# xiexh20/VisTracker

Measured on AMD Instinct MI355X. Metric: frames/sec joint SMPL+object fit, higher is better.
Workload: dtype f32 (decoder GEMMs: 22-bit split-f16 operands x3 MFMA, fp32 accumulate)

## Files before the change

include/vistracker.h:

```cpp
#ifndef VISTRACKER_H
#define VISTRACKER_H

#ifdef __cplusplus
extern "C" {
#endif

#define VT_OK 0
#define VT_ERR_ARG -1
#define VT_ERR_HIP -2
#define VT_ERR_BUSY -3

#define VT_SMPL_V 6890
#define VT_SMPL_J 52
#define VT_SMPL_NB 10
#define VT_SMPL_NP 459
#define VT_FEAT 611
#define VT_HID 128

const char *vt_last_error(void);
int vt_version(void);

typedef struct vt_smplh vt_smplh;

int vt_smplh_create(vt_smplh **out, const float *v_template, const float *shapedirs, const float *posedirs,
                    const float *J_regressor, const float *weights, const int *parents, void *stream);
void vt_smplh_destroy(vt_smplh *h);

long vt_smplh_workspace_floats(int B);

int vt_smplh_forward(const vt_smplh *h, const float *pose, const float *betas, const float *trans, int B,
                     float *verts, float *jtr, float *v_posed, float *ws, void *stream);

long vt_smplh_bwd_scratch_floats(int B);
int vt_smplh_backward(const vt_smplh *h, const float *pose, const float *betas, int B, const float *dverts,
                      const float *djtr, const float *v_posed, const float *ws, float *scratch,
                      float *dpose, float *dbetas, float *dtrans, void *stream);

long vt_smplh_prefix_floats(int B);
int vt_smplh_prefix(const vt_smplh *h, const float *pose, int B, float *ws, float *prefix, void *stream);
int vt_smplh_forward_prefixed(const vt_smplh *h, const float *pose, const float *betas, const float *trans, int B, const float *prefix,
                              float *verts, float *jtr, float *v_posed, float *ws, void *stream);
int vt_smplh_backward_free(const vt_smplh *h, const float *pose, int B, const float *dverts, const float *djtr, const float *v_posed,
                           const float *ws, float *scratch, int n_free_pose_cols, float *dpose, float *dbetas, float *dtrans, void *stream);

int vt_rodrigues_forward(const float *aa, int n, float *R, void *stream);
int vt_rodrigues_backward(const float *aa, int n, const float *dR, float *daa, void *stream);

typedef struct vt_landmarks vt_landmarks;
int vt_landmarks_create(vt_landmarks **out, const int *indptr, const int *indices, const float *data, int K, int V,
                        void *stream);
void vt_landmarks_destroy(vt_landmarks *h);
int vt_landmarks_forward(const vt_landmarks *h, const float *verts, int B, float *out, void *stream);
int vt_landmarks_backward(const vt_landmarks *h, const float *dout, int B, float *dverts, int accumulate, void *stream);

int vt_mahalanobis(const float *x, int B, int stride, int off, int n, const float *mean, const float *prec,
                   float *value, float *dx, float gscale, void *stream);

int vt_fill_f64(double *p, long n, double value, void *stream);
int vt_sum_to_term(const float *value, int n, float scale, double *term, void *stream);

typedef struct vt_sifnet vt_sifnet;
int vt_sifnet_create(vt_sifnet **out, const float *const *w, const float *const *b, const float *cam, void *stream);
void vt_sifnet_destroy(vt_sifnet *h);

int vt_nchw_to_nhwc(const float *src, int B, int C, int H, int W, float *dst, void *stream);

typedef struct {
    const float *maps[8];
    int res[8];
    const float *proj;
    int proj_cols;
    int act_level;
    int proj_level;
    int force_fp32;
} vt_maps;

int vt_query_forward(const vt_sifnet *h, const vt_maps *maps, const float *pts, const float *crop_center,
                     const float *body_center, int B, int N,
                     float *df, float *pca, float *parts, float *centers, float *vis, void *stream);
int vt_query_backward(const vt_sifnet *h, const vt_maps *maps, const float *pts, const float *crop_center,
                      const float *body_center, int B, int N,
                      const float *d_df, const float *d_pca, const float *d_parts, const float *d_centers,
                      const float *d_vis, float *dpts, void *stream);

long vt_query_projection_floats(const vt_maps *maps, int B);
int vt_query_build_projection(const vt_sifnet *h, const vt_maps *maps, int B, float *proj, void *stream);

int vt_query_human_loss(const vt_sifnet *h, const vt_maps *maps, const float *pts, const float *crop_center,
                        const float *body_center, int B, int N, const int *labels, const int *order, float w_dfh, float w_part,
                        float *dpts, double *terms, void *stream);
int vt_query_object_loss(const vt_sifnet *h, const vt_maps *maps, const float *pts, const float *crop_center,
                         const float *body_center, int B, int N, const float *occ, float w_obj,
                         float *dpts, double *terms, void *stream);

typedef struct vt_conv3x3 vt_conv3x3;
int vt_conv3x3_create(vt_conv3x3 **out, const float *weight, int cout, int cin, void *stream);
// ... 263 lines not shown
```

vistracker_amd/_lib.py:

```python
from __future__ import annotations

import ctypes as C
import os

_HERE = os.path.dirname(os.path.abspath(__file__))
LIB_PATH = os.environ.get("VT_LIB_PATH", os.path.join(_HERE, "libvistracker_hip.so"))

vp = C.c_void_p
fp = C.c_void_p
ci = C.c_int
cl = C.c_long
cf = C.c_float
cd = C.c_double


class VtMaps(C.Structure):
    _fields_ = [("maps", C.c_void_p * 8), ("res", C.c_int * 8), ("proj", C.c_void_p), ("proj_cols", C.c_int),
                ("act_level", C.c_int), ("proj_level", C.c_int), ("force_fp32", C.c_int)]


SIGNATURES = {
    "vt_last_error": (C.c_char_p, []),
    "vt_version": (ci, []),
    "vt_smplh_create": (ci, [C.POINTER(vp), vp, vp, vp, vp, vp, vp, vp]),
    "vt_smplh_destroy": (None, [vp]),
    "vt_smplh_workspace_floats": (cl, [ci]),
    "vt_smplh_bwd_scratch_floats": (cl, [ci]),
    "vt_smplh_forward": (ci, [vp, fp, fp, fp, ci, fp, fp, fp, fp, vp]),
    "vt_smplh_backward": (ci, [vp, fp, fp, ci, fp, fp, fp, fp, fp, fp, fp, fp, vp]),
    "vt_smplh_prefix_floats": (cl, [ci]),
    "vt_smplh_prefix": (ci, [vp, fp, ci, fp, fp, vp]),
    "vt_smplh_forward_prefixed": (ci, [vp, fp, fp, fp, ci, fp, fp, fp, fp, fp, vp]),
    "vt_smplh_backward_free": (ci, [vp, fp, ci, fp, fp, fp, fp, fp, ci, fp, fp, fp, vp]),
    "vt_rodrigues_forward": (ci, [fp, ci, fp, vp]),
    "vt_rodrigues_backward": (ci, [fp, ci, fp, fp, vp]),
    "vt_landmarks_create": (ci, [C.POINTER(vp), vp, vp, vp, ci, ci, vp]),
    "vt_landmarks_destroy": (None, [vp]),
    "vt_landmarks_forward": (ci, [vp, fp, ci, fp, vp]),
    "vt_landmarks_backward": (ci, [vp, fp, ci, fp, ci, vp]),
    "vt_mahalanobis": (ci, [fp, ci, ci, ci, ci, fp, fp, fp, fp, cf, vp]),
    "vt_fill_f64": (ci, [fp, cl, cd, vp]),
    "vt_sum_to_term": (ci, [fp, ci, cf, fp, vp]),
    "vt_sifnet_create": (ci, [C.POINTER(vp), C.POINTER(vp), C.POINTER(vp), vp, vp]),
    "vt_sifnet_destroy": (None, [vp]),
    "vt_nchw_to_nhwc": (ci, [fp, ci, ci, ci, ci, fp, vp]),
    "vt_query_forward": (ci, [vp, C.POINTER(VtMaps), fp, fp, fp, ci, ci, fp, fp, fp, fp, fp, vp]),
    "vt_query_backward": (ci, [vp, C.POINTER(VtMaps), fp, fp, fp, ci, ci, fp, fp, fp, fp, fp, fp, vp]),
    "vt_query_human_loss": (ci, [vp, C.POINTER(VtMaps), fp, fp, fp, ci, ci, fp, fp, cf, cf, fp, fp, vp]),
    "vt_query_object_loss": (ci, [vp, C.POINTER(VtMaps), fp, fp, fp, ci, ci, fp, cf, fp, fp, vp]),
    "vt_query_set_human_kernel": (ci, [ci]),
    "vt_sifnet_set_precision": (ci, [vp, ci]),
    "vt_sifnet_get_precision": (ci, [vp]),
    "vt_groupnorm_nhwc": (ci, [fp, fp, fp, ci, ci, ci, ci, cf, ci, fp, fp, vp]),
    "vt_upsample2x_bicubic_add": (ci, [fp, fp, ci, ci, ci, ci, fp, vp]),
    "vt_conv3x3_create": (ci, [C.POINTER(vp), vp, ci, ci, vp]),
    "vt_conv3x3_destroy": (None, [vp]),
    "vt_conv3x3_forward": (ci, [vp, fp, ci, ci, ci, fp, ci, ci, vp]),
    "vt_conv3x3_forward_gn": (ci, [vp, fp, ci, ci, fp, fp, fp, ci, ci, ci, ci, fp, ci, ci, vp]),
    "vt_groupnorm_stats": (ci, [fp, ci, ci, ci, ci, ci, ci, cf, fp, vp]),
    "vt_groupnorm_workspace_doubles": (C.c_long, [ci, ci, ci, ci]),
    "vt_groupnorm_finalize": (ci, [fp, ci, ci, ci, ci, ci, cf, vp]),
    "vt_conv3x3_tiles": (ci, [ci, ci]),
    "vt_kpts_step": (ci, [vp, fp, fp, fp, ci, ci, vp, cf, cf, fp, fp, fp, ci, vp]),
    "vt_query_human_step": (ci, [vp, C.POINTER(VtMaps), fp, fp, fp, ci, ci, fp, fp, cf, cf, ci, cf, fp, fp, fp, vp]),
    "vt_objstep_head": (ci, [fp, fp, fp, fp, ci, fp, ci, fp, fp, ci, fp, fp, fp, ci, fp, vp]),
    "vt_temporal_loss2": (ci, [fp, ci, ci, cf, fp, cf, fp, fp, ci, vp]),
    "vt_objstep_tail": (ci, [fp, ci, fp, fp, ci, fp, fp, ci, fp, fp, fp, fp, cf, fp, fp, fp, fp,
                             fp, fp, fp, cf, fp, fp, fp, cf, ci, cf, cf, cf,
                             fp, vp, ci, cf, ci, fp, fp, fp, ci, fp, ci, fp, vp]),
    "vt_objstep_tail_temporal": (ci, [fp, cf, fp, cf, fp, ci,
                                      fp, ci, fp, fp, ci, fp, fp, ci, fp, fp, fp, fp, cf, fp, fp, fp, fp,
                                      fp, fp, fp, cf, fp, fp, fp, cf, ci, cf, cf, cf,
                                      fp, vp, ci, cf, ci, fp, fp, fp, ci, fp, ci, fp, vp]),
    "vt_smplstep_tail": (ci, [fp, fp, fp, ci, fp, fp, cf, fp, cf, fp,
                              fp, ci, fp, ci, fp, fp, ci, cf, fp, ci, fp, ci, fp, fp, ci, cf, fp, ci, fp, ci, fp, fp, ci, cf, ci, cf, cf, cf,
                              fp, vp, ci, cf, ci, fp, fp, fp, ci, fp, ci, vp]),
    "vt_stream_set_skip_flag": (ci, [vp, vp]),
    "vt_conv1x1_create": (ci, [C.POINTER(vp), vp, vp, ci, ci, vp]),
    "vt_stem7x7_create": (ci, [C.POINTER(vp), vp, vp, ci, ci, vp]),
    "vt_stem7x7_destroy": (None, [vp]),
    "vt_stem7x7_forward": (ci, [vp, fp, ci, ci, ci, ci, ci, fp, ci, ci, vp]),
    "vt_conv1x1_destroy": (None, [vp]),
    "vt_conv1x1_forward": (ci, [vp, fp, ci, ci, fp, fp, fp, ci, ci, ci, ci, fp, ci, ci, fp, ci, ci, fp, ci, vp]),
    "vt_conv3x3_forward_block": (ci, [vp, fp, ci, ci, fp, fp, fp, ci, ci, ci, ci, fp, ci, ci, fp, ci, ci, fp, ci, ci, fp, ci, vp]),
    "vt_conv3x3_forward_block_stats": (ci, [vp, fp, ci, ci, fp, fp, fp, ci, ci, ci, ci, fp, ci, ci, fp, ci, ci, fp, ci, ci, fp, ci, fp, ci, vp]),
    "vt_avgpool2x2_stats": (ci, [fp, ci, ci, ci, ci, fp, fp, ci, vp]),
# ... 152 lines not shown
```

vistracker_amd/csrc/smplh.hip:

```cpp
#include "common.h"
#include <cstring>

#define V_ VT_SMPL_V
#define J_ VT_SMPL_J
#define NB_ VT_SMPL_NB
#define NP_ VT_SMPL_NP
#define VP_ 6912
#define NVT_ 27
#define KQ_ 472
#define NQ_ 480
#define J_LIVE_ 22
#define NP_LIVE_ ((J_LIVE_ - 1) * 9)
#define KF_ 272
#define NT_LIVE_ 13
#define NQ_HAND_ (NT_LIVE_ * 16)
#define NP_NUM_ (J_ * 3)
__host__ __device__ constexpr int kq_of_posemap(int p) { return p < NP_LIVE_ ? KF_ + p : p - NP_LIVE_; }
__host__ __device__ constexpr int nq_of_posemap(int p) { return p < NP_LIVE_ ? p : NQ_HAND_ + (p - NP_LIVE_); }
#define KQ_BETA0 (KF_ + NP_LIVE_)
#define KQ_TEMPLATE (KQ_ - 1)
#define NQ_BETA0 NP_LIVE_
static_assert(KF_ % 8 == 0 && KF_ >= NP_ - NP_LIVE_ && KQ_BETA0 + NB_ <= KQ_TEMPLATE && (KQ_ - KF_) % 8 == 0, "K order of Q_kcv");
static_assert(NQ_BETA0 + NB_ <= NQ_HAND_ && NQ_HAND_ + (NP_ - NP_LIVE_) <= NQ_, "N order of Q_t");
typedef float f32x4 __attribute__((ext_vector_type(4)));
#define MFMA16(a, b, c) __builtin_amdgcn_mfma_f32_16x16x4f32((a), (b), (c), 0, 0, 0)

#define WS_R 0
#define WS_J (52 * 9)
#define WS_G (WS_J + 52 * 3)
#define WS_A (WS_G + 52 * 12)
#define WS_FRAME (WS_A + 52 * 12)
#define PT_DA 0
#define PT_DTR 624
#define PT_N 627
#define KTOT_ (VP_ * 3)
#define KG_SLAB 24
#define NKS_ (KTOT_ / 16 / KG_SLAB)

#define SCHED_STEPS 32
#define SCHED_WIDTH 10
struct SmplParents { int p[J_]; int nsteps; short sched[SCHED_STEPS][SCHED_WIDTH]; };

#define SP_K 8
struct vt_smplh {
    float *Q_kcv, *Q_t, *W_jv, *W_v64, *J_t, *J_s;
    float *W_sp;
    int nnz;
    SmplParents par;
};

struct RodCtx { float n, ax, ay, az, c, s, qn, w, x, y, z; };

__device__ __forceinline__ void rodrigues_fwd(const float *t, float *R, RodCtx *k)
{
    const float xe = t[0] + 1e-8f, ye = t[1] + 1e-8f, ze = t[2] + 1e-8f;
    const float n = sqrtf(xe * xe + ye * ye + ze * ze);
    const float ax = t[0] / n, ay = t[1] / n, az = t[2] / n;
    const float h = n * 0.5f;
    const float c = cosf(h), s = sinf(h);
    const float q0 = c, q1 = s * ax, q2 = s * ay, q3 = s * az;
    const float qn = sqrtf(q0 * q0 + q1 * q1 + q2 * q2 + q3 * q3);
    const float w = q0 / qn, x = q1 / qn, y = q2 / qn, z = q3 / qn;
    const float w2 = w * w, x2 = x * x, y2 = y * y, z2 = z * z;
    const float wx = w * x, wy = w * y, wz = w * z, xy = x * y, xz = x * z, yz = y * z;
    R[0] = w2 + x2 - y2 - z2; R[1] = 2 * xy - 2 * wz;   R[2] = 2 * wy + 2 * xz;
    R[3] = 2 * wz + 2 * xy;   R[4] = w2 - x2 + y2 - z2; R[5] = 2 * yz - 2 * wx;
    R[6] = 2 * xz - 2 * wy;   R[7] = 2 * wx + 2 * yz;   R[8] = w2 - x2 - y2 + z2;
    if (k) { k->n = n; k->ax = ax; k->ay = ay; k->az = az; k->c = c; k->s = s; k->qn = qn; k->w = w; k->x = x; k->y = y; k->z = z; }
}

__device__ __forceinline__ void rodrigues_bwd(const float *t, const float *dR, float *dt)
{
    float R[9]; RodCtx k; rodrigues_fwd(t, R, &k);
    const float w = k.w, x = k.x, y = k.y, z = k.z;
    const float dw = 2 * w * (dR[0] + dR[4] + dR[8]) + 2 * (-z * dR[1] + y * dR[2] + z * dR[3] - x * dR[5] - y * dR[6] + x * dR[7]);
    const float dx = 2 * x * (dR[0] - dR[4] - dR[8]) + 2 * (y * dR[1] + z * dR[2] + y * dR[3] - w * dR[5] + z * dR[6] + w * dR[7]);
    const float dy = 2 * y * (-dR[0] + dR[4] - dR[8]) + 2 * (x * dR[1] + w * dR[2] + x * dR[3] + z * dR[5] - w * dR[6] + z * dR[7]);
    const float dz = 2 * z * (-dR[0] - dR[4] + dR[8]) + 2 * (-w * dR[1] + x * dR[2] + w * dR[3] + y * dR[5] + x * dR[6] + y * dR[7]);
    const float dot = w * dw + x * dx + y * dy + z * dz;
    const float dq0 = (dw - w * dot) / k.qn, dq1 = (dx - x * dot) / k.qn, dq2 = (dy - y * dot) / k.qn, dq3 = (dz - z * dot) / k.qn;
    const float dh = -k.s * dq0 + k.c * (k.ax * dq1 + k.ay * dq2 + k.az * dq3);
    const float dax = k.s * dq1, day = k.s * dq2, daz = k.s * dq3;
    const float dn = 0.5f * dh - (t[0] * dax + t[1] * day + t[2] * daz) / (k.n * k.n);
    dt[0] = dax / k.n + dn * (t[0] + 1e-8f) / k.n;
    dt[1] = day / k.n + dn * (t[1] + 1e-8f) / k.n;
    dt[2] = daz / k.n + dn * (t[2] + 1e-8f) / k.n;
}

__global__ void rodrigues_fwd_kernel(const float *aa, int n, float *R)
{
    const int i = blockIdx.x * blockDim.x + threadIdx.x;
    if (i >= n) return;
    float t[3] = {aa[3 * i], aa[3 * i + 1], aa[3 * i + 2]}, r[9];
    rodrigues_fwd(t, r, nullptr);
#pragma unroll
    for (int e = 0; e < 9; e++) R[9 * i + e] = r[e];
}

__global__ void rodrigues_bwd_kernel(const float *aa, int n, const float *dR, float *daa)
{
    const int i = blockIdx.x * blockDim.x + threadIdx.x;
// ... 255 lines not shown
            sdT[tid * 13 + r * 4 + 0] = dv[r] * vp[0]; sdT[tid * 13 + r * 4 + 1] = dv[r] * vp[1];
            sdT[tid * 13 + r * 4 + 2] = dv[r] * vp[2]; sdT[tid * 13 + r * 4 + 3] = dv[r];
        }
        __syncthreads();
        {
            f32x4 t[4];
#pragma unroll
            for (int mt = 0; mt < 4; mt++) t[mt] = (f32x4){0.f, 0.f, 0.f, 0.f};
#pragma unroll
            for (int ks = 0; ks < 13; ks++) {
                const float bv = j < 12 ? sA[f * 624 + (4 * ks + q) * 12 + j] : 0.f;
#pragma unroll
                for (int mt = 0; mt < 4; mt++) t[mt] = MFMA16(w1[mt][ks], bv, t[mt]);
            }
            const int r4 = (j < 12 ? (j >> 2) : 0) * 4 + 3;
#pragma unroll
            for (int mt = 0; mt < 4; mt++) {
#pragma unroll
                for (int r = 0; r < 4; r++) {
                    const int vl = 64 * wave + 16 * mt + 4 * q + r;
                    float x = t[mt][r] * sdT[vl * 13 + r4];
                    x += __shfl_down(x, 4, 16) + __shfl_down(x, 8, 16);
                    if (j < 3 && b < B) dvp_g[(size_t)b * KTOT_ + (size_t)(v0 + vl) * 3 + j] = x;
                }
            }
        }
        {
            f32x4 acc = (f32x4){0.f, 0.f, 0.f, 0.f}, acc2 = (f32x4){0.f, 0.f, 0.f, 0.f};
#pragma unroll
            for (int ks = 0; ks < 64; ks += 2) {
                const int va = 4 * ks + q, vb = va + 4;
                const float a0 = j < 12 ? sdT[va * 13 + j] : 0.f, a1 = j < 12 ? sdT[vb * 13 + j] : 0.f;
                acc = MFMA16(a0, w2[ks], acc);
                acc2 = MFMA16(a1, w2[ks + 1], acc2);
            }
            acc += acc2;
            if (b < B) {
                float *dst = part + ((size_t)tile * B + b) * PT_N;
                const int jn = wave * 16 + j;
#pragma unroll
                for (int r = 0; r < 4; r++) {
                    const int e = 4 * q + r;
                    if (e < 12) {
                        if (jn < J_) dst[PT_DA + jn * 12 + e] = acc[r];
                        else if (jn == J_ && (e & 3) == 3) dst[PT_DTR + (e >> 2)] = acc[r];
                    }
                }
            }
        }
        __syncthreads();
    }
}

#define BL_M 96
#ifndef BL_NW
#define BL_NW 1
#endif
#define BL_AS 132
__global__ __launch_bounds__(256) void smplh_bwd_blend_kernel(const float *__restrict__ Q_p, const float *__restrict__ dvp_g, int B, int ntiles,
                                                              float *__restrict__ part3, const int *skip)
{
    VT_SKIP_RETURN(skip);
    __shared__ __attribute__((aligned(16))) float sA[BL_M * BL_AS];
    const int tid = threadIdx.x, wave = tid >> 6, lane = tid & 63, q = lane >> 4, j = lane & 15;
    const int ks = blockIdx.x, m0 = blockIdx.z * BL_M, nt0 = blockIdx.y * (4 * BL_NW) + wave * BL_NW;
    const bool has_tile = nt0 < ntiles;
    f32x4 acc[6][BL_NW];
#pragma unroll
    for (int mt = 0; mt < 6; mt++)
#pragma unroll
        for (int n = 0; n < BL_NW; n++) acc[mt][n] = (f32x4){0.f, 0.f, 0.f, 0.f};
    const float4 *Q4 = reinterpret_cast<const float4 *>(Q_p);
#pragma unroll 1
    for (int c = 0; c < KG_SLAB / 8; c++) {
        __syncthreads();
        for (int i = tid; i < BL_M * 32; i += 256) {
            const int row = i >> 5, c4 = i & 31, b = m0 + row;
            float4 v = make_float4(0.f, 0.f, 0.f, 0.f);
            if (b < B) v = *reinterpret_cast<const float4 *>(dvp_g + (size_t)b * KTOT_ + (size_t)(ks * KG_SLAB + c * 8) * 16 + c4 * 4);
            *reinterpret_cast<float4 *>(sA + row * BL_AS + c4 * 4) = v;
        }
        __syncthreads();
        if (!has_tile) continue;
#pragma unroll
        for (int g = 0; g < 8; g++) {
            const size_t kg = (size_t)ks * KG_SLAB + c * 8 + g;
            float bq[BL_NW][4];
#pragma unroll
            for (int n = 0; n < BL_NW; n++) {
                const float4 fq = Q4[(kg * (NQ_ / 16) + min(nt0 + n, ntiles - 1)) * 64 + lane];
                bq[n][0] = fq.x; bq[n][1] = fq.y; bq[n][2] = fq.z; bq[n][3] = fq.w;
            }
#pragma unroll
            for (int mt = 0; mt < 6; mt++) {
                const float4 a4 = *reinterpret_cast<const float4 *>(sA + (mt * 16 + j) * BL_AS + g * 16 + q * 4);
                const float av[4] = {a4.x, a4.y, a4.z, a4.w};
#pragma unroll
                for (int s = 0; s < 4; s++)
#pragma unroll
                    for (int n = 0; n < BL_NW; n++) acc[mt][n] = MFMA16(av[s], bq[n][s], acc[mt][n]);
            }
        }
    }
#pragma unroll
    for (int mt = 0; mt < 6; mt++) {
#pragma unroll
        for (int r = 0; r < 4; r++) {
            const int b = m0 + mt * 16 + 4 * q + r;
            if (b < B) {
                float *dst = part3 + ((size_t)ks * B + b) * NQ_;
#pragma unroll
                for (int n = 0; n < BL_NW; n++)
                    if (nt0 + n < ntiles) dst[(nt0 + n) * 16 + j] = acc[mt][n][r];
            }
        }
    }
}

__global__ __launch_bounds__(256) void smplh_bwd_frame_kernel(const float *__restrict__ pose, const float *__restrict__ J_s,
                                                              SmplParents par, const float *__restrict__ ws,
                                                              const float *__restrict__ part, const float *__restrict__ part3,
                                                              const float *__restrict__ djtr, int B, int n_free, float *__restrict__ dpose,
                                                              float *__restrict__ dbetas, float *__restrict__ dtrans, const int *skip)
{
    VT_SKIP_RETURN(skip);
    __shared__ float red[PT_N], red3[NQ_];
    __shared__ float sdG[J_ * 12], sdJ[J_ * 3], sdR[J_ * 9];
    __shared__ float sG[J_ * 12], sRm[J_ * 9], sJr[J_ * 3];
    const int b = blockIdx.x, tid = threadIdx.x;
    const float *w = ws + (size_t)b * WS_FRAME;
    for (int i = tid; i < J_ * 12; i += 256) sG[i] = w[WS_G + i];
    for (int i = tid; i < J_ * 9; i += 256) sRm[i] = w[WS_R + i];
    for (int i = tid; i < J_ * 3; i += 256) sJr[i] = w[WS_J + i];
    for (int i = tid; i < PT_N; i += 256) {
        float s = 0.f;
#pragma unroll 9
        for (int t = 0; t < NVT_; t++) s += part[((size_t)t * B + b) * PT_N + i];
        red[i] = s;
    }
    const int ncol = n_free < NP_NUM_ ? NQ_HAND_ : NQ_, jfree = n_free / 3;
    for (int i = tid; i < ncol; i += 256) {
        float s = 0.f;
#pragma unroll 9
        for (int t = 0; t < NKS_; t++) s += part3[((size_t)t * B + b) * NQ_ + i];
        red3[i] = s;
    }
    __syncthreads();
    if (tid < J_) {
        const int j = tid;
        const float *G = sG + 12 * j; const float *Jr = sJr;
        float dj[3] = {0.f, 0.f, 0.f};
#pragma unroll
        for (int r = 0; r < 3; r++) {
            const float dat = red[PT_DA + 12 * j + r * 4 + 3];
#pragma unroll
            for (int c = 0; c < 3; c++) { sdG[12 * j + r * 4 + c] = red[PT_DA + 12 * j + r * 4 + c] - dat * Jr[3 * j + c]; dj[c] -= G[r * 4 + c] * dat; }
            sdG[12 * j + r * 4 + 3] = dat + (djtr ? djtr[(b * J_ + j) * 3 + r] : 0.f);
        }
// ... 88 lines not shown
            }
        }
    }
    float *W_v64 = new float[(size_t)VP_ * 64]();
    for (int v = 0; v < V_; v++) { for (int j = 0; j < J_; j++) { W_jv[(size_t)j * VP_ + v] = weights[(size_t)v * J_ + j]; W_v64[(size_t)v * 64 + j] = weights[(size_t)v * J_ + j]; } W_v64[(size_t)v * 64 + J_] = 1.0f; }
    float *W_sp = new float[(size_t)2 * SP_K * VP_]();
    int nnz = 0;
    for (int v = 0; v < V_; v++) {
        int k = 0;
        for (int j = 0; j < J_; j++) {
            const float w = weights[(size_t)v * J_ + j];
            if (w == 0.0f) continue;
            if (k < SP_K) { const int jj = j; memcpy(&W_sp[(size_t)k * VP_ + v], &jj, 4); W_sp[(size_t)(SP_K + k) * VP_ + v] = w; }
            k++;
        }
        nnz = k > nnz ? k : nnz;
    }
    h->nnz = nnz <= SP_K ? (nnz > 0 ? nnz : 1) : 0;
    for (int j = 0; j < J_; j++) for (int c = 0; c < 3; c++) {
        double a = 0; double sb[NB_] = {0};
        for (int v = 0; v < V_; v++) {
            const double r = J_regressor[(size_t)j * V_ + v];
            if (r == 0.0) continue;
            a += r * v_template[v * 3 + c];
            for (int l = 0; l < NB_; l++) sb[l] += r * shapedirs[((size_t)v * 3 + c) * NB_ + l];
        }
        J_t[j * 3 + c] = (float)a;
        for (int l = 0; l < NB_; l++) J_s[(j * 3 + c) * NB_ + l] = (float)sb[l];
    }
    int rc = VT_OK;
    if ((rc = vt_upload(&h->Q_kcv, Q_kcv, (size_t)KQ_ * 3 * VP_, st)) || (rc = vt_upload(&h->Q_t, Q_t, (size_t)VP_ * 3 * NQ_, st)) ||
        (rc = vt_upload(&h->W_jv, W_jv, (size_t)J_ * VP_, st)) || (rc = vt_upload(&h->W_v64, W_v64, (size_t)VP_ * 64, st)) ||
        (rc = vt_upload(&h->J_t, J_t, (size_t)J_ * 3, st)) || (rc = vt_upload(&h->J_s, J_s, (size_t)J_ * 3 * NB_, st)) ||
        (rc = vt_upload(&h->W_sp, W_sp, (size_t)2 * SP_K * VP_, st))) {
        return rc;
    }
    VT_HIP(hipStreamSynchronize(st));
    delete[] Q_kcv; delete[] Q_t; delete[] W_jv; delete[] W_v64; delete[] J_t; delete[] J_s; delete[] W_sp;
    *out = h;
    return VT_OK;
}

extern "C" void vt_smplh_destroy(vt_smplh *h)
{
    if (!h) return;
    hipFree(h->Q_kcv); hipFree(h->Q_t); hipFree(h->W_jv); hipFree(h->W_v64); hipFree(h->J_t); hipFree(h->J_s); hipFree(h->W_sp);
    delete h;
}

extern "C" long vt_smplh_workspace_floats(int B) { return (long)B * WS_FRAME; }
extern "C" long vt_smplh_bwd_scratch_floats(int B) { return (long)NVT_ * B * PT_N + (long)B * KTOT_ + (long)NKS_ * B * NQ_; }

#define BWD_FB 6

extern "C" long vt_smplh_prefix_floats(int B) { return (long)((B + FWD_FB - 1) / FWD_FB) * (VP_ / 64) * 3 * 256 * 4; }

#define FWD_LDS_FLOATS(w_) (FWD_R0 + FWD_FB * 64 * 3 + (w_) + FWD_FB * 3)
static int smplh_forward_launch(int mode, const vt_smplh *h, const float *pose, const float *betas, const float *trans, int B, float *verts, float *jtr,
                                float *v_posed, float *ws, float *prefix, hipStream_t st)
{
    const int *skip = mode == 1 ? nullptr : vt_skip_flag_of(st);
    hipLaunchKernelGGL(smplh_pose_kernel, dim3(B), dim3(64), 0, st, pose, betas, trans, h->J_t, h->J_s, h->par, ws, jtr, mode == 1 ? J_LIVE_ : 0,
                       mode == 2 ? J_LIVE_ : J_, mode == 1 ? 0 : 1, skip);
    VT_LAUNCH_CHECK();
    const size_t lds_f = sizeof(float) * FWD_LDS_FLOATS(h->nnz > 0 ? 2 * SP_K * 64 : J_ * 64), lds_max = sizeof(float) * FWD_LDS_FLOATS(J_ * 64);
    const dim3 grid(VP_ / 64, (B + FWD_FB - 1) / FWD_FB);
    if (mode == 0) {
        VT_LDS_LIMIT(smplh_verts_kernel<0>, lds_max);
        hipLaunchKernelGGL(smplh_verts_kernel<0>, grid, dim3(256), lds_f, st, h->Q_kcv, h->W_jv, betas, trans, ws, B, verts, v_posed, h->W_sp, h->nnz, prefix, skip);
    } else if (mode == 1) {
        VT_LDS_LIMIT(smplh_verts_kernel<1>, sizeof(float) * FWD_R0);
        hipLaunchKernelGGL(smplh_verts_kernel<1>, grid, dim3(256), sizeof(float) * FWD_R0, st, h->Q_kcv, h->W_jv, betas, trans, ws, B, verts, v_posed, h->W_sp,
                           h->nnz, prefix, skip);
    } else {
        VT_LDS_LIMIT(smplh_verts_kernel<2>, lds_max);
        hipLaunchKernelGGL(smplh_verts_kernel<2>, grid, dim3(256), lds_f, st, h->Q_kcv, h->W_jv, betas, trans, ws, B, verts, v_posed, h->W_sp, h->nnz, prefix, skip);
    }
    VT_LAUNCH_CHECK();
    return VT_OK;
}

extern "C" int vt_smplh_forward(const vt_smplh *h, const float *pose, const float *betas, const float *trans, int B,
                                float *verts, float *jtr, float *v_posed, float *ws, void *stream)
{
    VT_REQUIRE(h && pose && betas && trans && verts && v_posed && ws && B > 0, "vt_smplh_forward: null argument or B <= 0");
    return smplh_forward_launch(0, h, pose, betas, trans, B, verts, jtr, v_posed, ws, nullptr, vt_stream(stream));
}

extern "C" int vt_smplh_prefix(const vt_smplh *h, const float *pose, int B, float *ws, float *prefix, void *stream)
{
    VT_REQUIRE(h && pose && ws && prefix && B > 0, "vt_smplh_prefix: null argument or B <= 0");
    return smplh_forward_launch(1, h, pose, nullptr, nullptr, B, nullptr, nullptr, nullptr, ws, prefix, vt_stream(stream));
}

extern "C" int vt_smplh_forward_prefixed(const vt_smplh *h, const float *pose, const float *betas, const float *trans, int B, const float *prefix,
                                         float *verts, float *jtr, float *v_posed, float *ws, void *stream)
{
    VT_REQUIRE(h && pose && betas && trans && prefix && verts && v_posed && ws && B > 0, "vt_smplh_forward_prefixed: null argument or B <= 0");
    return smplh_forward_launch(2, h, pose, betas, trans, B, verts, jtr, v_posed, ws, const_cast<float *>(prefix), vt_stream(stream));
}

static int smplh_backward_launch(const vt_smplh *h, const float *pose, int B, const float *dverts, const float *djtr, const float *v_posed, const float *ws,
                                 float *scratch, int n_free, float *dpose, float *dbetas, float *dtrans, hipStream_t st)
{
    const int *skip = vt_skip_flag_of(st);
    const size_t lds = sizeof(float) * (256 * 13 + BWD_FB * 624);
    float *dvp_g = scratch + (size_t)NVT_ * B * PT_N, *part3 = dvp_g + (size_t)B * KTOT_;
    const int ntiles = n_free < NP_NUM_ ? NT_LIVE_ : NQ_ / 16;
    VT_LDS_LIMIT(smplh_bwd_tile_kernel<BWD_FB>, lds);
    hipLaunchKernelGGL(smplh_bwd_tile_kernel<BWD_FB>, dim3(NVT_, (B + BWD_FB - 1) / BWD_FB), dim3(256), lds, st, h->W_v64, ws, v_posed, dverts, B, scratch, dvp_g, skip);
    VT_LAUNCH_CHECK();
    hipLaunchKernelGGL(smplh_bwd_blend_kernel, dim3(NKS_, (ntiles + 4 * BL_NW - 1) / (4 * BL_NW), (B + BL_M - 1) / BL_M), dim3(256), 0, st, h->Q_t, dvp_g, B, ntiles,
                       part3, skip);
    VT_LAUNCH_CHECK();
    hipLaunchKernelGGL(smplh_bwd_frame_kernel, dim3(B), dim3(256), 0, st, pose, h->J_s, h->par, ws, scratch, part3, djtr, B, n_free, dpose, dbetas, dtrans, skip);
    VT_LAUNCH_CHECK();
    return VT_OK;
}

extern "C" int vt_smplh_backward(const vt_smplh *h, const float *pose, const float *betas, int B, const float *dverts,
                                 const float *djtr, const float *v_posed, const float *ws, float *scratch,
                                 float *dpose, float *dbetas, float *dtrans, void *stream)
{
    (void)betas;
    VT_REQUIRE(h && pose && dverts && v_posed && ws && scratch && dpose && dbetas && dtrans && B > 0, "vt_smplh_backward: null argument or B <= 0");
    return smplh_backward_launch(h, pose, B, dverts, djtr, v_posed, ws, scratch, NP_NUM_, dpose, dbetas, dtrans, vt_stream(stream));
}

extern "C" int vt_smplh_backward_free(const vt_smplh *h, const float *pose, int B, const float *dverts, const float *djtr, const float *v_posed,
                                      const float *ws, float *scratch, int n_free_pose_cols, float *dpose, float *dbetas, float *dtrans, void *stream)
{
    VT_REQUIRE(h && pose && dverts && v_posed && ws && scratch && dpose && dbetas && dtrans && B > 0, "vt_smplh_backward_free: null argument or B <= 0");
    VT_REQUIRE(n_free_pose_cols > 0 && n_free_pose_cols <= 3 * J_LIVE_ && n_free_pose_cols % 3 == 0,
               "vt_smplh_backward_free: n_free_pose_cols=%d must be a multiple of 3 in (0, %d] (the joints from %d on are the frozen ones of the layout)",
               n_free_pose_cols, 3 * J_LIVE_, J_LIVE_);
    return smplh_backward_launch(h, pose, B, dverts, djtr, v_posed, ws, scratch, n_free_pose_cols, dpose, dbetas, dtrans, vt_stream(stream));
}

extern "C" int vt_rodrigues_forward(const float *aa, int n, float *R, void *stream)
{
    VT_REQUIRE(aa && R && n > 0, "vt_rodrigues_forward: bad argument");
    hipLaunchKernelGGL(rodrigues_fwd_kernel, dim3((n + 255) / 256), dim3(256), 0, vt_stream(stream), aa, n, R);
    VT_LAUNCH_CHECK();
    return VT_OK;
}

extern "C" int vt_rodrigues_backward(const float *aa, int n, const float *dR, float *daa, void *stream)
{
    VT_REQUIRE(aa && dR && daa && n > 0, "vt_rodrigues_backward: bad argument");
    hipLaunchKernelGGL(rodrigues_bwd_kernel, dim3((n + 255) / 256), dim3(256), 0, vt_stream(stream), aa, n, dR, daa);
    VT_LAUNCH_CHECK();
    return VT_OK;
}
```

vistracker_amd/fitting.py:

```python
from __future__ import annotations

import contextlib
import ctypes as C
import functools
import os
import threading
import time
from dataclasses import dataclass, field

import numpy as np
import torch

from . import _lib as L
from . import ops

FIT_WEIGHTS = {"pose": 1e-5, "hand": 1e-5, "j2d": 0.09, "object": 900.0, "part": 0.0025, "contact": 900.0, "scale": 100.0,
               "df_h": 100.0, "mask": 0.0009, "ocent": 0.0, "pinit": 25.0, "rot": 100.0, "trans": 100.0,
               "stemp": 10000.0, "otemp": 225.0, "ovtemp": 2500.0, "collide": 9.0}
SMPLT_WEIGHTS = {"pose": 1e-5, "hand": 1e-5, "kpts": 0.09, "temp": 900.0, "ptemp": 25.0, "pinit": 900.0}
JOINT_WEIGHTS_66 = np.repeat(np.array([1, 10, 10, 10, 5, 5, 10, 1, 1, 10, 1, 1, 5, 5, 5, 5, 5, 5, 1, 1, 1, 1], np.float32), 3)
JOINT_WEIGHTS_66[37:39] = 10.0


def _lib():
# ... 186 lines not shown

class _SmplFit(_Fit):

    def __init__(self, pose, betas, trans, names, nsteps, prev_loss, prof=None, smpl=None):
        dev = pose.device; B = self.B = pose.shape[0]
        super().__init__(dev, names, nsteps, prev_loss, prof)
        self.pose, self.betas, self.trans = pose, betas, trans
        self.verts = torch.empty(B, 6890, 3, device=dev); self.jtr = torch.empty(B, 52, 3, device=dev); self.vposed = torch.empty_like(self.verts)
        self.ws = torch.empty(_lib().vt_smplh_workspace_floats(B), device=dev); self.scratch = torch.empty(_lib().vt_smplh_bwd_scratch_floats(B), device=dev)
        self.dverts = torch.empty_like(self.verts); self.J = torch.empty(B, 25, 3, device=dev); self.dJ = torch.empty_like(self.J)
        self.dpose = torch.empty(B, 156, device=dev); self.dbetas = torch.empty(B, 10, device=dev); self.dtrans = torch.empty(B, 3, device=dev)
        self.vb = torch.empty(B, device=dev)
        self.pose_init = pose.clone()
        self.prefix, self.n_free = None, 156
        if smpl is not None:
            self.prefix = torch.empty(_lib().vt_smplh_prefix_floats(B), device=dev); self.n_free = 66
            _chk(_lib().vt_smplh_prefix(smpl.h, pose.data_ptr(), B, self.ws.data_ptr(), self.prefix.data_ptr(), L.stream_ptr()))
            self.dpose.zero_()

    @property
    def vert_order_ptr(self):
        return self.vert_order.data_ptr() if self.vert_order is not None else None


class _ObjectFit(_Fit):

    def __init__(self, ctx, obj_R, obj_t, sil, nsteps, prof):
        dev = obj_R.device; B = self.B = obj_R.shape[0]; N = self.N = ctx.obj_points.shape[0]; NV = self.NV = ctx.obj_verts.shape[0]
        super().__init__(dev, ["object", "otemp", "ovtemp", "mask", "trans", "contact", "collide", "scale"], nsteps, 300.0, prof)
        self.obj_R, self.obj_t, self.sil = obj_R, obj_t, sil
        self.R = torch.empty(B, 3, 3, device=dev); self.X = torch.empty(B, N, 3, device=dev); self.dX = torch.empty_like(self.X)
        self.svd_ws = torch.empty(B, 22, device=dev)
        self.dR = torch.empty(B, 3, 3, device=dev); self.dM = torch.empty(B, 3, 3, device=dev); self.dt = torch.empty(B, 3, device=dev)
        if sil is not None:
            self.Vt = torch.empty(B, NV, 3, device=dev); self.dVt = torch.empty_like(self.Vt)
            self.fidx = torch.empty(B, sil.size, sil.size, dtype=torch.int32, device=dev); self.dimg = torch.empty(B, sil.size, sil.size, device=dev)
            self.sws = torch.empty(_lib().vt_sil_workspace_floats(B, NV, ctx.obj_faces.shape[0], sil.size), device=dev)
            if not ctx.fused_steps:
                self.img = torch.empty_like(self.dimg); self.per = torch.empty(B, device=dev)
        self.trans_init = None
        self.Vc = self.cws = None
        self.contact = None


class FitContext:
    use_projection = True
    sort_object_points = True
    sort_query_points = True
    collision_loss = False
    fused_steps = os.environ.get("VT_FUSED_STEPS", "1") != "0"
    fused_smpl_query = os.environ.get("VT_FUSED_SMPL_QUERY", "0") != "0"
    device_skip = os.environ.get("VT_DEVICE_SKIP", "1") != "0"
    frozen_hands = True

    def __init__(self, smpl_model, regressors, priors, decoders=None, part_labels=None, obj_verts=None, obj_faces=None, obj_points=None,
                 cam=ops.DEFAULT_CAM, device="cuda:0"):
        self.device = torch.device(device)
        dev = self.device
        self.smpl = ops.SmplhHandle(smpl_model, dev)
        self.b25 = ops.LandmarkHandle(regressors["body25"], dev)
        self.net = ops.SifNetHandle(decoders, cam, dev) if decoders is not None else None
        self.cam = np.ascontiguousarray(cam, np.float32)
        t = lambda a, dt=torch.float32: None if a is None else torch.as_tensor(np.ascontiguousarray(a), dtype=dt, device=dev)
        self.pri = {k: t(v) for k, v in priors.items()}
        self.labels = t(part_labels, torch.int32)
        self.vert_order = t(morton_order(np.asarray(smpl_model["v_template"])), torch.int32) if self.sort_query_points else None
        if obj_points is not None and self.sort_object_points:
            obj_points = np.asarray(obj_points, np.float32)[morton_order(obj_points)]
        self.obj_verts = t(obj_verts); self.obj_faces = t(obj_faces, torch.int32); self.obj_points = t(obj_points)
        self.smpl_faces = t(np.asarray(smpl_model["f"]).astype(np.int32), torch.int32) if "f" in smpl_model else None
        self.jw66 = t(JOINT_WEIGHTS_66)

    range_retries = 0
    fp32_fallbacks = 0
    _counter_lock = threading.Lock()
    host_wait_s = 0.0

    def _with_range_fallback(self, maps, params, run):
        if self.net is None or maps is None or maps.force_fp32 or self.net.precision == "fp32":
            return run()
        saved = [p.clone() for p in params]
        while True:
            try:
                return run()
            except FloatingPointError as e:
                import warnings
                for p, s0 in zip(params, saved):
                    p.copy_(s0)
                if maps.act_level + 1 < maps.ACT_LEVELS:
                    maps.set_act_level(maps.act_level + 1)
                    warnings.warn(f"{e}; repeating the fit at operand-range level {maps.act_level} of the split-f16 decoders", RuntimeWarning)
                    with self._counter_lock:
                        self.range_retries += 1
                    continue
                if maps.force_fp32:
                    raise
                warnings.warn(f"{e}; repeating the fit on the strict-fp32 decoder kernels (5x slower)", RuntimeWarning)
                maps.set_force_fp32(True)
                with self._counter_lock:
                    self.fp32_fallbacks += 1
                return run()

    def smpl_forward(self, pose, betas, trans, verts, jtr, vposed, ws, prefix=None):
        if prefix is not None:
            _chk(_lib().vt_smplh_forward_prefixed(self.smpl.h, pose.data_ptr(), betas.data_ptr(), trans.data_ptr(), pose.shape[0], prefix.data_ptr(),
                                                  verts.data_ptr(), jtr.data_ptr(), vposed.data_ptr(), ws.data_ptr(), L.stream_ptr()))
            return
        _chk(_lib().vt_smplh_forward(self.smpl.h, pose.data_ptr(), betas.data_ptr(), trans.data_ptr(), pose.shape[0], verts.data_ptr(),
                                     jtr.data_ptr(), vposed.data_ptr(), ws.data_ptr(), L.stream_ptr()))

    def smpl_backward(self, pose, betas, dverts, vposed, ws, scratch, dpose, dbetas, dtrans, n_free=156):
        if n_free < 156:
            _chk(_lib().vt_smplh_backward_free(self.smpl.h, pose.data_ptr(), pose.shape[0], dverts.data_ptr(), None, vposed.data_ptr(), ws.data_ptr(),
                                               scratch.data_ptr(), n_free, dpose.data_ptr(), dbetas.data_ptr(), dtrans.data_ptr(), L.stream_ptr()))
            return
        _chk(_lib().vt_smplh_backward(self.smpl.h, pose.data_ptr(), betas.data_ptr(), pose.shape[0], dverts.data_ptr(), None, vposed.data_ptr(),
                                      ws.data_ptr(), scratch.data_ptr(), dpose.data_ptr(), dbetas.data_ptr(), dtrans.data_ptr(), L.stream_ptr()))

    def hand_prior_value(self, pose, terms, name, scratch_b):
        B = pose.shape[0]
        for off, m, p in ((66, "lhand_mean", "lhand_prec"), (111, "rhand_mean", "rhand_prec")):
            _chk(_lib().vt_mahalanobis(pose.data_ptr(), B, 156, off, 45, self.pri[m].data_ptr(), self.pri[p].data_ptr(), scratch_b.data_ptr(), None, 0.0, L.stream_ptr()))
            _chk(_lib().vt_sum_to_term(scratch_b.data_ptr(), B, 1.0 / 45.0, terms.ptr(name), L.stream_ptr()))

    def body_prior(self, pose, dpose, w, terms, name, scratch_b):
        B = pose.shape[0]
        _chk(_lib().vt_mahalanobis(pose.data_ptr(), B, 156, 3, 63, self.pri["body_mean"].data_ptr(), self.pri["body_prec"].data_ptr(),
                                   scratch_b.data_ptr(), dpose.data_ptr(), w / B, L.stream_ptr()))
        _chk(_lib().vt_sum_to_term(scratch_b.data_ptr(), B, 1.0 / B, terms.ptr(name), L.stream_ptr()))

    def _run_fit(self, f, start, end, check_every, outer, prof=None):
        res = FitResult()
        with self._skip_after_stop(f.stop) as skipping:
            watch = _StopWatch(self, f.stop, skipping)
            for it in range(start, end):
                step, phase, w, armed = outer(it)
                for i in range(10):
                    step(f, phase, (it - start) * 10 + i, w, armed)
                res.steps += 10
                res.outer_iters += 1
                if (it - start) % check_every == check_every - 1 and watch.check():
                    res.stopped_early = True
                    break
            res.stopped_early = res.stopped_early or watch.final()
        res.losses = f.hist.cpu().numpy()
        if res.stopped_early:
            res.steps = int(np.isfinite(res.losses).sum())
            res.outer_iters = -(-res.steps // 10)
        _flush_events(prof, f.lp, res.steps if (res.stopped_early and self.device_skip) else None)
        _check_finite(res, "fit")
        return res

    def fit_smplt(self, pose, betas, trans, kpts, max_iter=100, iter_for_global=8, temporal=True, pinit_w=900.0,
                  lr_global=0.01, lr_all=0.001, it_range=None, check_every=1, weights=None, early_stop=True):
        with torch.cuda.device(pose.device):
            return self._fit_smplt(pose, betas, trans, kpts, max_iter, iter_for_global, temporal, pinit_w, lr_global, lr_all, it_range, check_every, weights, early_stop)

    def _fit_smplt(self, pose, betas, trans, kpts, max_iter, iter_for_global, temporal, pinit_w, lr_global, lr_all, it_range, check_every, weights, early_stop=True):
        _require_params(pose, betas, trans)
        table = dict(SMPLT_WEIGHTS); table["pinit"] = pinit_w
        if weights is not None:
            table.update({k: float(v) for k, v in weights.items() if k in table})
        start, end = it_range if it_range is not None else (0, max_iter)
        f = _SmplFit(pose, betas, trans, ["kpts", "temp", "ptemp", "pose", "pinit", "hand"], (end - start) * 10, 0.0,
                     smpl=self.smpl if self.frozen_hands else None)
        f.kpts = _as_input(kpts, pose.device)
        f.temporal = temporal and f.B >= 3
        self.hand_prior_value(pose, f.terms, "hand", f.vb)

        def outer(it):
            if f.adam is None or it == iter_for_global:
                if it < iter_for_global:
                    f.adam = AdamState([(trans, 3, f.dtrans, lr_global), (pose, 3, f.dpose, lr_global), (betas, 2, f.dbetas, lr_global)], f.stop)
                else:
                    f.adam = AdamState([(trans, 3, f.dtrans, lr_all), (pose, 66, f.dpose, lr_all), (betas, 10, f.dbetas, lr_all)], f.stop)
            return self._smplt_step, None, f.terms.weights(table, it // 3), int(early_stop and it > 0.3 * max_iter)
        return self._run_fit(f, start, end, check_every, outer)

    def optimize_smpl(self, maps, pose, betas, trans, crop_center, body_center, body_kpts, max_iter=100, iter_for_betas=1,
                      iter_for_pose=1, iter_for_kpts=1, it_range=None, net_size=512.0, check_every=1, prof=None, early_stop=True):
        with torch.cuda.device(pose.device):
            return self._with_range_fallback(maps, (pose, betas, trans), lambda: self._optimize_smpl(
                maps, pose, betas, trans, crop_center, body_center, body_kpts, max_iter, iter_for_betas, iter_for_pose, iter_for_kpts, it_range, net_size,
                check_every, prof, early_stop))

    def _optimize_smpl(self, maps, pose, betas, trans, crop_center, body_center, body_kpts, max_iter, iter_for_betas, iter_for_pose, iter_for_kpts,
                       it_range, net_size, check_every, prof, early_stop=True):
        dev = pose.device
        _require_params(pose, betas, trans)
        split_route = self.net.precision != "fp32" and not maps.force_fp32
        if self.use_projection and split_route:
            maps.build_projection(self.net)
        total = iter_for_betas + iter_for_kpts + iter_for_pose + max_iter
        start, end = it_range if it_range is not None else (0, total)
        f = _SmplFit(pose, betas, trans, ["df_h", "part", "pose", "pinit", "j2d", "stemp", "hand"], (end - start) * 10, 300.0, prof,
                     smpl=self.smpl if self.frozen_hands else None)
        f.maps, f.net_size = maps, net_size
        f.crop_center, f.body_center, f.body_kpts = _as_input(crop_center, dev), _as_input(body_center, dev), _as_input(body_kpts, dev)
        f.vert_order = self.vert_order
        if self.sort_query_points:
            self.smpl_forward(pose, betas, trans, f.verts, f.jtr, f.vposed, f.ws, f.prefix)
            v0 = f.verts[f.B // 2]
            f.vert_order = morton_order_device(torch.stack([v0[:, 0] / v0[:, 2], v0[:, 1] / v0[:, 2]], 1))
        self.hand_prior_value(pose, f.terms, "hand", f.vb)
        if not self.fused_steps:
            step = self._smpl_step
        elif split_route and self.fused_smpl_query:
            step = self._smpl_step_fused_query
        else:
            step = self._smpl_step_fused
        arm_after = 0.25 * max_iter + iter_for_betas + iter_for_pose

        def outer(it):
            if it < iter_for_betas:
                phase = "global"
                if f.adam is None:
                    f.adam = AdamState([(betas, 2, f.dbetas, 0.02), (trans, 3, f.dtrans, 0.02)], f.stop)
            else:
                phase = "kpts" if it >= iter_for_betas + iter_for_pose else "smpl all pose"
                if f.adam is None or it == iter_for_betas:
                    f.adam = AdamState([(trans, 3, f.dtrans, 0.006), (pose, 66, f.dpose, 0.006), (betas, 10, f.dbetas, 0.006)], f.stop)
            return step, phase, f.terms.weights(FIT_WEIGHTS, 1 if phase != "kpts" else it / 3), int(early_stop and it > arm_after)
        return self._run_fit(f, start, end, check_every, outer, prof)

    def optimize_smpl_object(self, maps, smpl_verts, obj_R, obj_t, obj_s, crop_center, body_center, occ, sil=None, noise=None,
                             iter_for_obj=15, iter_for_sil=30, joint_iter=10, max_iter=100, it_range=None, seed=0, check_every=1, prof=None, early_stop=True):
        with torch.cuda.device(obj_R.device):
            return self._with_range_fallback(maps, (obj_R, obj_t), lambda: self._optimize_smpl_object(
                maps, smpl_verts, obj_R, obj_t, obj_s, crop_center, body_center, occ, sil, noise, iter_for_obj, iter_for_sil, joint_iter, max_iter, it_range,
                seed, check_every, prof, early_stop))

    def _optimize_smpl_object(self, maps, smpl_verts, obj_R, obj_t, obj_s, crop_center, body_center, occ, sil, noise, iter_for_obj, iter_for_sil,
                              joint_iter, max_iter, it_range, seed, check_every, prof, early_stop=True):
        dev = obj_R.device; B = obj_R.shape[0]
        _require_params(obj_R, obj_t)
        if self.use_projection and self.net.precision != "fp32" and not maps.force_fp32:
            maps.build_projection(self.net, reuse=True)
        total = joint_iter + iter_for_obj + max_iter + iter_for_sil
        start, end = it_range if it_range is not None else (0, total)
        f = _ObjectFit(self, obj_R, obj_t, sil, (end - start) * 10, prof)
        f.maps = maps
        f.smpl_verts, f.obj_s, f.crop_center, f.body_center, f.occ = (_as_input(x, dev) for x in (smpl_verts, obj_s, crop_center, body_center, occ))
# ... 261 lines not shown
```

Baseline: 156.8.

## Add frame-packed SMPL-H backward tile kernel and shrink blend M tile

Adds a new backward tile kernel that packs four frames into the MFMA N dimension and keeps the skinning weights in registers across two frame groups. It also prefetches the next group's per-vertex data while the current group computes. This is meant to make better use of the MFMA units and cut the re-reading of W_v64 for every frame. Separately, the blend kernel's M tile drops from 96 to 32 rows. That creates more blocks at small batch sizes but loads the Q tiles more often. The packed path is on by default, with a runtime switch to fall back to the old kernel.

```diff
diff --git a/include/vistracker.h b/include/vistracker.h
--- a/include/vistracker.h
+++ b/include/vistracker.h
@@ -42,6 +42,9 @@
                               float *verts, float *jtr, float *v_posed, float *ws, void *stream);
 int vt_smplh_backward_free(const vt_smplh *h, const float *pose, int B, const float *dverts, const float *djtr, const float *v_posed,
                            const float *ws, float *scratch, int n_free_pose_cols, float *dpose, float *dbetas, float *dtrans, void *stream);
+
+int vt_smplh_set_backward_tile(vt_smplh *h, int packed);
+int vt_smplh_get_backward_tile(const vt_smplh *h);
 
 int vt_rodrigues_forward(const float *aa, int n, float *R, void *stream);
 int vt_rodrigues_backward(const float *aa, int n, const float *dR, float *daa, void *stream);
diff --git a/vistracker_amd/_lib.py b/vistracker_amd/_lib.py
--- a/vistracker_amd/_lib.py
+++ b/vistracker_amd/_lib.py
@@ -32,6 +32,8 @@
     "vt_smplh_prefix": (ci, [vp, fp, ci, fp, fp, vp]),
     "vt_smplh_forward_prefixed": (ci, [vp, fp, fp, fp, ci, fp, fp, fp, fp, fp, vp]),
     "vt_smplh_backward_free": (ci, [vp, fp, ci, fp, fp, fp, fp, fp, ci, fp, fp, fp, vp]),
+    "vt_smplh_set_backward_tile": (ci, [vp, ci]),
+    "vt_smplh_get_backward_tile": (ci, [vp]),
     "vt_rodrigues_forward": (ci, [fp, ci, fp, vp]),
     "vt_rodrigues_backward": (ci, [fp, ci, fp, fp, vp]),
     "vt_landmarks_create": (ci, [C.POINTER(vp), vp, vp, vp, ci, ci, vp]),
diff --git a/vistracker_amd/csrc/smplh.hip b/vistracker_amd/csrc/smplh.hip
--- a/vistracker_amd/csrc/smplh.hip
+++ b/vistracker_amd/csrc/smplh.hip
@@ -1,4 +1,5 @@
 #include "common.h"
+#include <atomic>
 #include <cstring>
 
 #define V_ VT_SMPL_V
@@ -47,6 +48,7 @@
     float *W_sp;
     int nnz;
     SmplParents par;
+    std::atomic<int> bwd_packed{1};
 };
 
 struct RodCtx { float n, ax, ay, az, c, s, qn, w, x, y, z; };
@@ -408,7 +410,132 @@
     }
 }
 
-#define BL_M 96
+#define PK_FB 4
+#define PK_TS 49
+template <int NG>
+__global__ __launch_bounds__(256, 2) void smplh_bwd_tile_packed_kernel(const float *__restrict__ W_v64, const float *__restrict__ ws,
+                                                                    const float *__restrict__ v_posed, const float *__restrict__ dverts,
+                                                                    int B, float *__restrict__ part, float *__restrict__ dvp_g, const int *skip)
+{
+    VT_SKIP_RETURN(skip);
+    extern __shared__ __attribute__((aligned(16))) float lds[];
+    float *sdT = lds;
+    float *sA = sdT + 256 * PK_TS;
+    const int tid = threadIdx.x, tile = blockIdx.x, b0 = blockIdx.y * (NG * PK_FB), v0 = tile * 256, v = v0 + tid;
+    const int wave = tid >> 6, lane = tid & 63, q = lane >> 4, j = lane & 15;
+    float w1[4][13], w2[64];
+#pragma unroll
+    for (int mt = 0; mt < 4; mt++)
+#pragma unroll
+        for (int ks = 0; ks < 13; ks++) w1[mt][ks] = W_v64[(size_t)(v0 + 64 * wave + 16 * mt + j) * 64 + 4 * ks + q];
+#pragma unroll
+    for (int ks = 0; ks < 64; ks++) w2[ks] = W_v64[(size_t)(v0 + 4 * ks + q) * 64 + wave * 16 + j];
+    float dvn[PK_FB][3], vpn[PK_FB][3];
+    auto fetch = [&](int bg) {
+#pragma unroll
+        for (int f = 0; f < PK_FB; f++) {
+#pragma unroll
+            for (int r = 0; r < 3; r++) { dvn[f][r] = 0.f; vpn[f][r] = 0.f; }
+            if (bg + f < B && v < V_) {
+                const size_t o = ((size_t)(bg + f) * V_ + v) * 3;
+                dvn[f][0] = dverts[o]; dvn[f][1] = dverts[o + 1]; dvn[f][2] = dverts[o + 2];
+                vpn[f][0] = v_posed[o]; vpn[f][1] = v_posed[o + 1]; vpn[f][2] = v_posed[o + 2];
+            }
+        }
+    };
+    fetch(b0);
+#pragma unroll 1
+    for (int g = 0; g < NG; g++) {
+        const int bg = b0 + g * PK_FB;
+        if (bg >= B) break;
+        for (int i = tid; i < PK_FB * 624; i += 256) {
+            const int f = i / 624, rem = i - 624 * f, jt = rem / 12, b = min(bg + f, B - 1);
+            sA[jt * 48 + 12 * f + (rem - 12 * jt)] = ws[(size_t)b * WS_FRAME + WS_A + rem];
+        }
+#pragma unroll
+        for (int f = 0; f < PK_FB; f++)
+#pragma unroll
+            for (int r = 0; r < 3; r++) {
+                float *d = sdT + tid * PK_TS + 12 * f + 4 * r;
+                d[0] = dvn[f][r] * vpn[f][0]; d[1] = dvn[f][r] * vpn[f][1]; d[2] = dvn[f][r] * vpn[f][2]; d[3] = dvn[f][r];
+            }
+        if (g + 1 < NG) fetch(bg + PK_FB);
+        __syncthreads();
+        const bool st0 = j < 3, st1 = st0 && bg + 1 < B, st2 = st0 && bg + 2 < B, st3 = j >= 4 && j < 7 && bg + 3 < B;
+        float *dbase = dvp_g + (size_t)bg * KTOT_ + (size_t)(v0 + 64 * wave + 4 * q) * 3 + (j < 3 ? j : j - 4);
+#pragma unroll
+        for (int mh = 0; mh < 2; mh++) {
+            f32x4 t[2][3];
+#pragma unroll
+            for (int mt = 0; mt < 2; mt++)
+#pragma unroll
+                for (int nt = 0; nt < 3; nt++) t[mt][nt] = (f32x4){0.f, 0.f, 0.f, 0.f};
+#pragma unroll
+            for (int ks = 0; ks < 13; ks++) {
+                float bv[3];
+#pragma unroll
+                for (int nt = 0; nt < 3; nt++) bv[nt] = sA[(4 * ks + q) * 48 + 16 * nt + j];
+#pragma unroll
+                for (int mt = 0; mt < 2; mt++)
+#pragma unroll
+                    for (int nt = 0; nt < 3; nt++) t[mt][nt] = MFMA16(w1[2 * mh + mt][ks], bv[nt], t[mt][nt]);
+            }
+#pragma unroll
+            for (int mt = 0; mt < 2; mt++) {
+#pragma unroll
+                for (int r = 0; r < 4; r++) {
+                    const int vl = 64 * wave + 16 * (2 * mh + mt) + 4 * q + r;
+                    const float *row = sdT + vl * PK_TS;
+                    const float x0 = t[mt][0][r] * row[j | 3], x1 = t[mt][1][r] * row[(16 + j) | 3], x2 = t[mt][2][r] * row[(32 + j) | 3];
+                    const float x0_4 = __shfl_down(x0, 4, 16), x0_8 = __shfl_down(x0, 8, 16), x0_12 = __shfl_down(x0, 12, 16);
+                    const float x1_4 = __shfl_down(x1, 4, 16), x1_8 = __shfl_down(x1, 8, 16), x1_12 = __shfl_down(x1, 12, 16);
+                    const float x2_4 = __shfl_down(x2, 4, 16), x2_8 = __shfl_down(x2, 8, 16);
+                    const float y0 = x0 + (x0_4 + x0_8), y1 = x0_12 + (x1 + x1_4), y2 = x1_8 + (x1_12 + x2), y3 = x2 + (x2_4 + x2_8);
+                    float *dst = dbase + (16 * (2 * mh + mt) + r) * 3;
+                    if (st0) dst[0] = y0;
+                    if (st1) dst[KTOT_] = y1;
+                    if (st2) dst[2 * KTOT_] = y2;
+                    if (st3) dst[3 * KTOT_] = y3;
+                }
+            }
+            __builtin_amdgcn_sched_barrier(0);
+        }
+        {
+            f32x4 acc[3], acc2[3];
+#pragma unroll
+            for (int mi = 0; mi < 3; mi++) { acc[mi] = (f32x4){0.f, 0.f, 0.f, 0.f}; acc2[mi] = (f32x4){0.f, 0.f, 0.f, 0.f}; }
+#pragma unroll
+            for (int ks = 0; ks < 64; ks += 2) {
+                const float *ra = sdT + (4 * ks + q) * PK_TS + j, *rb = ra + 4 * PK_TS;
+#pragma unroll
+                for (int mi = 0; mi < 3; mi++) {
+                    acc[mi] = MFMA16(ra[16 * mi], w2[ks], acc[mi]);
+                    acc2[mi] = MFMA16(rb[16 * mi], w2[ks + 1], acc2[mi]);
+                }
+            }
+            const int jn = wave * 16 + j;
+#pragma unroll
+            for (int mi = 0; mi < 3; mi++) {
+                acc[mi] += acc2[mi];
+#pragma unroll
+                for (int r = 0; r < 4; r++) {
+                    const int m = 16 * mi + 4 * q + r, f = m / 12, e = m - 12 * f, b = bg + f;
+                    if (b < B) {
+                        float *dst = part + ((size_t)tile * B + b) * PT_N;
+                        if (jn < J_) dst[PT_DA + jn * 12 + e] = acc[mi][r];
+                        else if (jn == J_ && (e & 3) == 3) dst[PT_DTR + (e >> 2)] = acc[mi][r];
+                    }
+                }
+            }
+        }
+        __syncthreads();
+    }
+}
+
+#ifndef BL_MT
+#define BL_MT 2
+#endif
+#define BL_M (16 * BL_MT)
 #ifndef BL_NW
 #define BL_NW 1
 #endif
@@ -421,9 +548,9 @@
     const int tid = threadIdx.x, wave = tid >> 6, lane = tid & 63, q = lane >> 4, j = lane & 15;
     const int ks = blockIdx.x, m0 = blockIdx.z * BL_M, nt0 = blockIdx.y * (4 * BL_NW) + wave * BL_NW;
     const bool has_tile = nt0 < ntiles;
-    f32x4 acc[6][BL_NW];
-#pragma unroll
-    for (int mt = 0; mt < 6; mt++)
+    f32x4 acc[BL_MT][BL_NW];
+#pragma unroll
+    for (int mt = 0; mt < BL_MT; mt++)
 #pragma unroll
         for (int n = 0; n < BL_NW; n++) acc[mt][n] = (f32x4){0.f, 0.f, 0.f, 0.f};
     const float4 *Q4 = reinterpret_cast<const float4 *>(Q_p);
@@ -448,7 +575,7 @@
                 bq[n][0] = fq.x; bq[n][1] = fq.y; bq[n][2] = fq.z; bq[n][3] = fq.w;
             }
 #pragma unroll
-            for (int mt = 0; mt < 6; mt++) {
+            for (int mt = 0; mt < BL_MT; mt++) {
                 const float4 a4 = *reinterpret_cast<const float4 *>(sA + (mt * 16 + j) * BL_AS + g * 16 + q * 4);
                 const float av[4] = {a4.x, a4.y, a4.z, a4.w};
 #pragma unroll
@@ -459,7 +586,7 @@
         }
     }
 #pragma unroll
-    for (int mt = 0; mt < 6; mt++) {
+    for (int mt = 0; mt < BL_MT; mt++) {
 #pragma unroll
         for (int r = 0; r < 4; r++) {
             const int b = m0 + mt * 16 + 4 * q + r;
@@ -654,6 +781,17 @@
 extern "C" long vt_smplh_bwd_scratch_floats(int B) { return (long)NVT_ * B * PT_N + (long)B * KTOT_ + (long)NKS_ * B * NQ_; }
 
 #define BWD_FB 6
+#ifndef BWD_PK_NG
+#define BWD_PK_NG 2
+#endif
+
+extern "C" int vt_smplh_set_backward_tile(vt_smplh *h, int packed)
+{
+    VT_REQUIRE(h && (packed == 0 || packed == 1), "vt_smplh_set_backward_tile: bad handle, or a form other than 0 (per frame) / 1 (frame-packed)");
+    h->bwd_packed.store(packed, std::memory_order_relaxed);
+    return VT_OK;
+}
+extern "C" int vt_smplh_get_backward_tile(const vt_smplh *h) { return h ? h->bwd_packed.load(std::memory_order_relaxed) : VT_ERR_ARG; }
 
 extern "C" long vt_smplh_prefix_floats(int B) { return (long)((B + FWD_FB - 1) / FWD_FB) * (VP_ / 64) * 3 * 256 * 4; }
 
@@ -706,11 +844,18 @@
                                  float *scratch, int n_free, float *dpose, float *dbetas, float *dtrans, hipStream_t st)
 {
     const int *skip = vt_skip_flag_of(st);
-    const size_t lds = sizeof(float) * (256 * 13 + BWD_FB * 624);
     float *dvp_g = scratch + (size_t)NVT_ * B * PT_N, *part3 = dvp_g + (size_t)B * KTOT_;
     const int ntiles = n_free < NP_NUM_ ? NT_LIVE_ : NQ_ / 16;
-    VT_LDS_LIMIT(smplh_bwd_tile_kernel<BWD_FB>, lds);
-    hipLaunchKernelGGL(smplh_bwd_tile_kernel<BWD_FB>, dim3(NVT_, (B + BWD_FB - 1) / BWD_FB), dim3(256), lds, st, h->W_v64, ws, v_posed, dverts, B, scratch, dvp_g, skip);
+    if (h->bwd_packed.load(std::memory_order_relaxed)) {
+        const size_t lds = sizeof(float) * (256 * PK_TS + J_ * 12 * PK_FB);
+        constexpr int fb = BWD_PK_NG * PK_FB;
+        VT_LDS_LIMIT(smplh_bwd_tile_packed_kernel<BWD_PK_NG>, lds);
+        hipLaunchKernelGGL(smplh_bwd_tile_packed_kernel<BWD_PK_NG>, dim3(NVT_, (B + fb - 1) / fb), dim3(256), lds, st, h->W_v64, ws, v_posed, dverts, B, scratch, dvp_g, skip);
+    } else {
+        const size_t lds = sizeof(float) * (256 * 13 + BWD_FB * 624);
+        VT_LDS_LIMIT(smplh_bwd_tile_kernel<BWD_FB>, lds);
+        hipLaunchKernelGGL(smplh_bwd_tile_kernel<BWD_FB>, dim3(NVT_, (B + BWD_FB - 1) / BWD_FB), dim3(256), lds, st, h->W_v64, ws, v_posed, dverts, B, scratch, dvp_g, skip);
+    }
     VT_LAUNCH_CHECK();
     hipLaunchKernelGGL(smplh_bwd_blend_kernel, dim3(NKS_, (ntiles + 4 * BL_NW - 1) / (4 * BL_NW), (B + BL_M - 1) / BL_M), dim3(256), 0, st, h->Q_t, dvp_g, B, ntiles,
                        part3, skip);
diff --git a/vistracker_amd/fitting.py b/vistracker_amd/fitting.py
--- a/vistracker_amd/fitting.py
+++ b/vistracker_amd/fitting.py
@@ -262,6 +262,7 @@
     fused_smpl_query = os.environ.get("VT_FUSED_SMPL_QUERY", "0") != "0"
     device_skip = os.environ.get("VT_DEVICE_SKIP", "1") != "0"
     frozen_hands = True
+    packed_smplh_backward = True
 
     def __init__(self, smpl_model, regressors, priors, decoders=None, part_labels=None, obj_verts=None, obj_faces=None, obj_points=None,
                  cam=ops.DEFAULT_CAM, device="cuda:0"):
@@ -311,6 +312,9 @@
                     self.fp32_fallbacks += 1
                 return run()
 
+    def _select_smplh_kernels(self):
+        _chk(_lib().vt_smplh_set_backward_tile(self.smpl.h, 1 if self.packed_smplh_backward else 0))
+
     def smpl_forward(self, pose, betas, trans, verts, jtr, vposed, ws, prefix=None):
         if prefix is not None:
             _chk(_lib().vt_smplh_forward_prefixed(self.smpl.h, pose.data_ptr(), betas.data_ptr(), trans.data_ptr(), pose.shape[0], prefix.data_ptr(),
@@ -368,6 +372,7 @@
 
     def _fit_smplt(self, pose, betas, trans, kpts, max_iter, iter_for_global, temporal, pinit_w, lr_global, lr_all, it_range, check_every, weights, early_stop=True):
         _require_params(pose, betas, trans)
+        self._select_smplh_kernels()
         table = dict(SMPLT_WEIGHTS); table["pinit"] = pinit_w
         if weights is not None:
             table.update({k: float(v) for k, v in weights.items() if k in table})
@@ -398,6 +403,7 @@
                        it_range, net_size, check_every, prof, early_stop=True):
         dev = pose.device
         _require_params(pose, betas, trans)
+        self._select_smplh_kernels()
         split_route = self.net.precision != "fp32" and not maps.force_fp32
         if self.use_projection and split_route:
             maps.build_projection(self.net)
```

Measured after the change: 157.9, median of 6. Within noise of the previous version (+0.7%).
